# kianoosh-j/CL_MultiView_Stereo

Hardware: AMD Instinct MI355X
Metric: Mpix/s depth (1080p, 128 depth hyp, 5 views) + depth L1 vs ref (higher is better)
Workload: dtype i8 (NCC: 8-bit intensities as int8 v_dot4 operands, i32 window sums, f32 costs; SLIC / superpixel SAD / refinement in f32 with the reference's f64 promotions)

## Files before the change

### cl_multiview_stereo_amd/csrc/launch_plan.cpp

```cpp
#include "launch_plan.h"

#include <algorithm>
#include <climits>
#include <cmath>
#include <cstdlib>
#include <cstring>

extern char** environ;

namespace mvs {
namespace plan {

Tuning plan_tuning() {
  Tuning t;
  bool any = false;
  for (char** e = environ; e && *e && !any; e++) {
    const char* s = *e;
    any = s[0] == 'M' && s[1] == 'V' && s[2] == 'S' && s[3] == '_' && (s[4] == 'S' || s[4] == 'F');
  }
  if (!any) return t;
  const auto num = [](const char* name, int dflt) {
    const char* e = getenv(name);
    return e ? atoi(e) : dflt;
  };
  const auto is = [](const char* name, const char* value) {
    const char* e = getenv(name);
    return e && !strcmp(e, value);
  };
  const int wps = num("MVS_SWEEP_WPS", 0);
  t.sweep_wps = (wps == 1 || wps == 2 || wps == 4) ? wps : 0;
  t.sweep_transpose = num("MVS_SWEEP_TRANSPOSE", 2);
  t.sweep_hz = num("MVS_SWEEP_HZ", 1) != 0;
  t.sweep_ring = num("MVS_SWEEP_RING", 1) != 0;
  t.sweep_ring_fast = num("MVS_SWEEP_RING_FAST", 1) != 0;
  if (const char* kv = getenv("MVS_SAD_KERNEL")) {
    t.sad_kernel = kv;
    t.sad_named = true;
  }
  t.sad_aff = getenv("MVS_SAD_AFF") == nullptr;
  t.filter_px = is("MVS_FILTER_KERNEL", "px");
  t.filter_fb_q = num("MVS_FILTER_FB", 2);
  t.filter_fb_px = num("MVS_FILTER_FB", 4);
  t.filter_ns = num("MVS_FILTER_NS", 2);
  t.filter_bound = num("MVS_FILTER_BOUND", 1) != 0;
  t.filter_ref_order = is("MVS_FILTER_ORDER", "ref");
  t.slic_tiles9 = num("MVS_SLIC_TILES9", 0) == 1;
  t.slic_update_walk = num("MVS_SLIC_UPDATE", 1) != 0;
  return t;
}

SlicPlan plan_slic(const Tuning& t, int V, int W, int H, int S, int no_iter, int edge_enable, int search,
                   int enforce_connectivity) {
  SlicPlan p;
  p.V = V, p.W = W, p.H = H, p.S = S;
  const int mw = p.mw = map_dim(W, S), mh = p.mh = map_dim(H, S);
  float xy = 1.0f / (1.4242f * (float)S);
  float col = 15.0f / (1.7321f * 128.0f);
  p.xy = xy * xy;
  p.col = col * col;
  const bool tiles = S % kLocal == 0;
  const int cpl = p.cpl = S * 3 / kLocal;
  const int G = p.G = tiles ? cpl * cpl : (int)__builtin_ceilf((float)(S * S * 9) / (float)(kLocal * kLocal));
  const int ntx = p.ntx = (W + 15) / 16, nty = p.nty = (H + 15) / 16;
  const size_t P = (size_t)V * W * H;
  const bool l16 = !tiles && no_iter > 0 && (long)mw * mh <= 65536;
  size_t sb = tiles ? sizeof(float) * 6 * (size_t)G * mw * mh * V : 0;
  if (enforce_connectivity || edge_enable) sb = std::max(sb, sizeof(uint32_t) * P);
  if (l16) sb = std::max(sb, sizeof(uint16_t) * P);
  p.scratch_bytes = sb;

  p.steps.reserve(6 + 2 * (size_t)no_iter);
  const auto step = [&p](SlicKernel k, unsigned gx, unsigned gy, unsigned gz, unsigned block) -> SlicStep& {
    p.steps.push_back(SlicStep{k, 0, 0, 0, 0, 0, {gx, gy, gz}, block, false, false, false, false});
    return p.steps.back();
  };
  const unsigned cx = (mw + 63) / 64, px = (W + 255) / 256;
  step(kSlicInitCenters, cx, mh, V, 64);
  if (edge_enable == 1 || edge_enable == 2) {
    step(kSlicEdge, px, H, V, 256);
    if (edge_enable == 1)
      step(kSlicEdgeStore, (unsigned)std::min<long>(((long)P + 255) / 256, 8192), 1, 1, 256);
    else
      step(kSlicApplyEdge, cx, mh, V, 64);
  }
  const bool tiles4 = !search && (S == 32 || S == 64) && (long)W * H * 16 < (1L << 31) &&
                      (long)mw * mh * G * 24 < (1L << 31) && !t.slic_tiles9;
  const auto assign = [&](bool more) {
    if (tiles) {
      SlicStep& s = tiles4 ? step(kSlicAssignTiles4, (ntx + 3) / 4, nty, V, 256)
                           : step(kSlicAssignTiles9, (ntx * nty + 3) / 4, V, 1, 256);
      if (tiles4)
        s.S16 = S / 16;
      else
        s.S3 = search;
      s.labels = !more, s.part = more;
    } else {
      SlicStep& s = step(kSlicAssign, (W + kAssignTW - 1) / kAssignTW, (H + kAssignTH - 1) / kAssignTH, V, 256);
      s.S3 = search;
      s.labels = !(more && l16), s.lb16 = more && l16;
    }
  };
  const bool walk = (long)W * H * 16 < (1L << 31) && t.slic_update_walk;
  assign(no_iter > 0);
  for (int i = 0; i < no_iter; i++) {
    if (tiles) {
      step(kSlicUpdateFinalize, (mw * mh + 31) / 32, V, 1, 256).CPL = cpl == 6 ? 6 : 0;
    } else {
      SlicStep& s = step(walk ? kSlicUpdateWalk : kSlicUpdate, (mw * mh + 3) / 4, V, 1, 256);
      s.UT = G > 4 ? 4 : 1;
      s.LT = l16 ? 16 : 32;
    }
    assign(i + 1 < no_iter);
  }
  if (enforce_connectivity) {
    step(kSlicSuppress, px, H, V, 256).to_scratch = true;
    step(kSlicSuppress, px, H, V, 256);
  }
  return p;
}

SpixlSweepPlan plan_sweep_spixl(const Tuning& t, int V, int W, int H, int S, int D, const float* levels,
                                const int* vs, const int* sn, int aw, int z0, int z1, bool allow_relayout) {
  SpixlSweepPlan p;
  if (z1 <= z0) return p;
  if ((long)(W + H) * H * 16 >= (1L << 31)) {
    p.err = "superpixel sweep: image too large for 32-bit offsets";
    return p;
  }
  p.launch = true;
  p.mw = map_dim(W, S);
  p.mh = map_dim(H, S);
  const long M = (long)p.mw * p.mh;
  const bool half = D <= 32;
  int wps = (D + 63) / 64;
  wps = wps >= 3 ? 4 : wps;
  const int wps_env = half ? 0 : t.sweep_wps;
  if (wps_env) wps = wps_env;
  const int tmode = t.sweep_transpose;
  p.tstride = H;
  if (tmode > 0 && allow_relayout) {
    std::vector<int32_t> slot(4 * (size_t)V, -1);
    long units = 0;
    for (int z = z0; z < z1; z++)
      for (int k = 0; k < sn[z]; k++) {
        const int v = vs[(size_t)V * z + k];
        if (v < 0 || v >= V) continue;
        const int dx = v % aw - z % aw, dy = v / aw - z / aw;
        const int kind = dx == 0 ? 1 : tmode < 2 ? 0 : dx == dy ? 2 : dx == -dy ? 3 : 0;
        if (kind && slot[4 * v + kind] < 0 && units + W + H <= INT32_MAX) {
          slot[4 * v + kind] = (int32_t)units;
          units += kind == 1 ? W : W + H - 1;
        }
      }
    if (units > 0) {
      for (int v = 0; v < V; v++)
        for (int kind = 1; kind < 4; kind++)
          if (slot[4 * v + kind] >= 0) p.relayouts.push_back({v, kind, slot[4 * v + kind]});
      p.slot = std::move(slot);
      p.units = units;
    }
  }
  const bool relaid = p.units > 0;
  bool hz = !relaid && t.sweep_hz;
  for (int z = z0; z < z1 && hz; z++)
    for (int k = 0; k < sn[z] && hz; k++) {
      const int v = vs[(size_t)V * z + k];
      if (v / aw != z / aw) hz = false;
      const float fdxv = (float)(v % aw - z % aw);
      for (int l = 0; l < D && hz; l++) {
        const float f = levels[l] * fdxv;
        if (!(fabsf(f) < 16777216.0f) || f != truncf(f)) hz = false;
      }
    }
  bool ring = hz && !half && t.sweep_ring;
  if (ring) {
    float rng = 0.0f;
    for (int c0 = 0; c0 < D; c0 += 64) {
      float lo = levels[c0], hi = lo;
      for (int l = c0; l < std::min(D, c0 + 64); l++) {
        lo = std::min(lo, levels[l]);
        hi = std::max(hi, levels[l]);
      }
      rng = std::max(rng, hi - lo);
    }
    int mdx = 0;
    for (int z = z0; z < z1; z++)
      for (int k = 0; k < sn[z]; k++) mdx = std::max(mdx, std::abs(vs[(size_t)V * z + k] % aw - z % aw));
    if (2.0 * (S - 1) + 2.0 + (double)rng * mdx + 1.0 > (double)kSwU) ring = false;
  }
  p.form = ring ? kSweepHzRing : relaid ? kSweepRelaid : hz ? kSweepHzGather : kSweepGeneral;
  p.lps = half ? 32 : 64;
  p.wps = ring ? (wps_env ? wps_env : 1) : wps;
  const int spb = half ? 8 : 4 / p.wps;
  const long nb = (M + spb - 1) / spb;
  p.grid_x = (unsigned)(8 * ((nb + 7) / 8));
  p.grid_y = (unsigned)(z1 - z0);
  const int last[5] = {p.form, p.lps, p.wps, tmode, (int)p.relayouts.size()};
  std::copy(last, last + 5, p.last);
  return p;
}

bool sad_band_geometry(int DC, int RR, bool aff, int V, int W, int H, int D, const float* levels, const int* vs,
                       const int* sn, int aw, float bl, int z, SadPlan& p) {
  const int TH = RR - 4, PPW = DC / 8;
  const int nn = sn[z];
  const int nch = (D + DC - 1) / DC;
  const int rx = z % aw, ry = z / aw;
  constexpr int RW = sizeof(SadRec) / 4;
  std::vector<int32_t> table((size_t)std::max(1, nch * nn) * RW, 0);
  int span_x = 0;
  float span_y = 0.0f;
  for (int c = 0; c < nch; c++)
    for (int n = 0; n < nn; n++) {
      SadRec e{};
      const int view = vs[V * z + n];
      const int dx = view % aw - rx, dy = view / aw - ry;
      e.view = view;
      e.sxmin = 1 << 30;
      e.sxmax = -(1 << 30);
      e.fdymin = INFINITY;
      e.fdymax = -INFINITY;
      for (int j = 0; j < DC; j++) {
        const int dl = std::min(c * DC + j, D - 1);
        const float d = levels[dl];
        const float fdx = d * (float)dx;
        const float fdy = (bl * d) * (float)dy;
        if (fdx != std::trunc(fdx) || std::fabs(fdx) > 1e6f) return false;
        e.sx[j] = (int)fdx;
        e.fdy[j] = fdy;
        if (fdy != std::trunc(fdy) || std::fabs(fdy) > 1e6f) aff = false;
        if (c * DC + j < D) {
          e.sxmin = std::min(e.sxmin, e.sx[j]);
          e.sxmax = std::max(e.sxmax, e.sx[j]);
          e.fdymin = std::min(e.fdymin, fdy);
          e.fdymax = std::max(e.fdymax, fdy);
        }
      }
      span_x = std::max(span_x, e.sxmax - e.sxmin);
      span_y = std::max(span_y, e.fdymax - e.fdymin);
      std::memcpy(table.data() + ((size_t)c * nn + n) * RW, &e, sizeof(SadRec));
    }
  SadArgs a{};
  a.W = W; a.H = H; a.D = D; a.nn = nn; a.z = z; a.nch = nch;
  a.bw = (64 + span_x + 63) & ~63;
  a.brows = RR + (int)std::ceil(span_y) + (aff ? 0 : 1);
  const size_t lds = 16 * 2 * (size_t)a.brows * a.bw + (aff ? 0 : 4 * 2 * (size_t)DC * RR);
  if (a.bw > 64 * SB_NBLK) return false;
  if (lds > 160 * 1024 || (size_t)4 * TH * 64 * 8 > 16 * 2 * (size_t)a.brows * a.bw) return false;
  a.tiles_x = (W + SB_TW - 1) / SB_TW;
  a.ntiles = a.tiles_x * ((H + TH - 1) / TH);
  a.tiles_per_xcd = (a.ntiles + 7) / 8;
  p.band = true;
  p.TH = TH;
  p.PPW = PPW;
  p.AFF = aff;
  p.BWT = aff ? (a.bw == 64 ? 64 : 128) : 0;
  p.table = std::move(table);
  p.args = a;
  p.lds = lds;
  p.grid_x = 8 * a.tiles_per_xcd;
  p.grid_y = 1;
  return true;
}

SadPlan plan_sad(const Tuning& t, int V, int W, int H, int D, const float* levels, const int* vs, const int* sn,
                 int aw, float bl, int z) {
  SadPlan p;
  const std::string& kind = t.sad_kernel;
  const bool try2 = kind == "auto" || kind == "sys8x2", try1 = kind == "auto" || kind == "sys8";
  if (try2 && sad_band_geometry(16, 12, t.sad_aff, V, W, H, D, levels, vs, sn, aw, bl, z, p)) return p;
  if (try1 && sad_band_geometry(8, 12, t.sad_aff, V, W, H, D, levels, vs, sn, aw, bl, z, p)) return p;
  if (t.sad_named && kind != "gather") {
    p.err = "k_sad_band variant " + kind + " cannot stage this geometry (MVS_SAD_KERNEL set explicitly)";
    return p;
  }
  p.grid_x = (W + PT - 1) / PT;
  p.grid_y = (H + PT - 1) / PT;
  return p;
}

FilterPlan plan_remove_incons(const Tuning& t, int V, int W, int H, int aw, int z0, int z1, int ya, int yb,
                              bool band) {
  FilterPlan p;
  const int NR = yb - ya;
  p.PP = band ? (long)NR * W : (long)W * H;
  p.proj_off = band ? -(long)ya * W : 0;
  if (z1 <= z0 || NR <= 0) return p;
  const unsigned gx = (W + 255) / 256;
  const auto grid = [&p](unsigned x, unsigned y, unsigned z) { p.grid[0] = x, p.grid[1] = y, p.grid[2] = z; };
  const bool off32 = (long)V * W * H * 4 < (1L << 31);
  if (V <= 8 && off32) {
    p.kernel = kFilterSel8;
    grid(gx, NR, z1 - z0);
  } else if (V <= 16) {
    p.kernel = kFilterPx16_8;
    grid(gx, NR, 1);
  } else if (V <= 32 && off32 && !t.filter_px) {
    p.kernel = kFilterQ;
    p.FB = t.filter_fb_q == 4 ? 4 : 2;
    p.NS = t.filter_ns == 1 ? 1 : 2;
    p.ROWB = aw % p.FB == 0;
    p.RM = !t.filter_ref_order;
    p.inb = (V % aw == 0 && t.filter_bound) ? 1 : 0;
    const unsigned tx = (W + 63) / 64, groups = (z1 - z0 + kFilterRG - 1) / kFilterRG;
    if (p.RM)
      grid(tx * groups, NR, 1);
    else
      grid(tx, NR, groups);
    p.block = 64 * kFilterRG;
  } else if (V <= 32) {
    p.kernel = kFilterPx32;
    p.FB = t.filter_fb_px == 4 ? 4 : t.filter_fb_px == 2 ? 2 : 8;
    grid(gx, NR, 1);
  } else if (V <= 64 && off32) {
    p.kernel = kFilterSel64;
    grid(gx, NR, z1 - z0);
  } else {
    p.kernel = kFilterPlain;
    grid(gx, NR, z1 - z0);
  }
  return p;
}

SgmPlan plan_sgm(int W, int H, int D, int path) {
  SgmPlan p;
  if (W < 1 || H < 1 || D < 1 || path < 0 || path > 3) {
    p.err = "sgm: bad dimensions or path";
    return p;
  }
  if (D > kSgmMaxD) {
    p.err = "sgm: more than 16384 levels";
    return p;
  }
  const bool vertical = path >= 2;
  p.rev = path & 1;
  p.n = vertical ? H : W;
  p.lines = vertical ? W : H;
// ... 106 lines not shown
```

### cl_multiview_stereo_amd/csrc/launch_plan.h

```cpp
#pragma once
#include <cstddef>
#include <cstdint>
#include <string>
#include <vector>

namespace mvs {

inline int map_dim(int n, int S) {
  return (int)__builtin_ceilf((float)n / (float)S);
}

constexpr int kLocal = 16;
constexpr int kAssignTW = 64, kAssignTH = 16;

constexpr int kSwU = 336;

struct SweepArgs {
  int V, W, H, mw, mh, D, aw, z;
  float bl;
};
constexpr float SB_INIT = 1000000.0f;

constexpr int SB_TW = 60;
constexpr int SB_NBLK = 2;
struct SadArgs {
  int W, H, D, nn, z;
  int tiles_x, ntiles, tiles_per_xcd, nch;
  int bw, brows;
};
struct alignas(16) SadRec {
  int view, sxmin, sxmax, pad0;
  float fdymin, fdymax;
  int pad1[2];
  int sx[16];
  float fdy[16];
};
static_assert(sizeof(SadRec) == 160, "SadRec is uploaded as 40 int32 words");
constexpr int PT = 32;

constexpr int kFilterRG = 4;

namespace plan {

struct Tuning {
  bool slic_tiles9 = false;
  bool slic_update_walk = true;
  int sweep_wps = 0;
  int sweep_transpose = 2;
  bool sweep_hz = true;
  bool sweep_ring = true;
  bool sweep_ring_fast = true;
  std::string sad_kernel = "auto";
  bool sad_named = false;
  bool sad_aff = true;
  bool filter_px = false;
  int filter_fb_q = 2;
  int filter_fb_px = 4;
  int filter_ns = 2;
  bool filter_bound = true;
  bool filter_ref_order = false;
};
Tuning plan_tuning();

enum SlicKernel {
  kSlicInitCenters, kSlicEdge, kSlicEdgeStore, kSlicApplyEdge,
  kSlicAssign,
  kSlicAssignTiles9,
  kSlicAssignTiles4,
  kSlicUpdateFinalize,
  kSlicUpdateWalk,
  kSlicUpdate,
  kSlicSuppress
};
struct SlicStep {
  SlicKernel kernel;
  int S3, S16, CPL, UT, LT;
  unsigned grid[3], block;
  bool labels;
  bool lb16;
  bool part;
  bool to_scratch;
};
struct SlicPlan {
  int V = 0, W = 0, H = 0, S = 0;
  int mw = 0, mh = 0;
  float xy = 0, col = 0;
  int G = 0, cpl = 0, ntx = 0, nty = 0;
  size_t scratch_bytes = 0;
  std::vector<SlicStep> steps;
};
SlicPlan plan_slic(const Tuning& t, int V, int W, int H, int S, int no_iter, int edge_enable, int search,
                   int enforce_connectivity);

constexpr int kSweepGeneral = 0, kSweepHzGather = 1, kSweepHzRing = 2, kSweepRelaid = 3;
struct SpixlRelayout {
  int view, kind, slot;
};
struct SpixlSweepPlan {
  const char* err = nullptr;
  bool launch = false;
  int form = 0, lps = 64, wps = 1;
  int mw = 0, mh = 0;
  unsigned grid_x = 0, grid_y = 0;
  std::vector<int32_t> slot;
  std::vector<SpixlRelayout> relayouts;
  long units = 0, tstride = 0;
  int last[5] = {0, 0, 0, 0, 0};
};
SpixlSweepPlan plan_sweep_spixl(const Tuning& t, int V, int W, int H, int S, int D, const float* levels,
                                const int* vs, const int* sn, int aw, int z0, int z1, bool allow_relayout);

struct SadPlan {
  bool band = false;
  int TH = 0, PPW = 0, AFF = 0, BWT = 0;
  std::vector<int32_t> table;
  SadArgs args{};
  size_t lds = 0;
  unsigned grid_x = 0, grid_y = 1;
  std::string err;
};
bool sad_band_geometry(int DC, int RR, bool aff, int V, int W, int H, int D, const float* levels, const int* vs,
                       const int* sn, int aw, float bl, int z, SadPlan& p);
SadPlan plan_sad(const Tuning& t, int V, int W, int H, int D, const float* levels, const int* vs, const int* sn,
                 int aw, float bl, int z);

enum FilterKernel { kFilterNone, kFilterSel8, kFilterPx16_8, kFilterQ, kFilterPx32, kFilterSel64, kFilterPlain };
struct FilterPlan {
  FilterKernel kernel = kFilterNone;
  int FB = 0, NS = 0, ROWB = 0, RM = 0;
  int inb = 0;
  unsigned grid[3] = {0, 1, 1}, block = 256;
  long PP = 0;
  long proj_off = 0;
};
FilterPlan plan_remove_incons(const Tuning& t, int V, int W, int H, int aw, int z0, int z1, int ya, int yb,
                              bool band);

constexpr int kSgmLanes = 0, kSgmColumns = 1;
constexpr int kSgmMaxLpl = 16;
constexpr int kSgmLanesOneWave = 64 * kSgmMaxLpl;
constexpr int kSgmColumnsLpw = 16;
constexpr int kSgmColumnsMaxD = 16 * kSgmColumnsLpw;
constexpr int kSgmMaxD = 16 * kSgmLanesOneWave;
struct SgmPlan {
  const char* err = nullptr;
  int form = kSgmLanes;
  int lpl = 1;
  int waves = 1;
  bool vec = false;
  int n = 0, lines = 0;
  int sstride = 0, lstride = 0;
  int sx = 0;
  bool rev = false;
  unsigned grid = 0, block = 0;
  size_t lds = 0;
};
SgmPlan plan_sgm(int W, int H, int D, int path);

constexpr int kSgmSheared = 2;
constexpr int sgm_diag_x0(int g, int lane, int H, int sx) { return sx > 0 ? 64 * g - (H - 1) + lane : 64 * g + lane; }
constexpr int sgm_diag_ylo(int g, int W, int H, int sx) {
  const int y = sx > 0 ? H - 1 - 64 * g - 63 : 64 * g - (W - 1);
  return y > 0 ? y : 0;
}
constexpr int sgm_diag_yhi(int g, int W, int H, int sx) {
  const int y = sx > 0 ? W + H - 2 - 64 * g : 64 * g + 63;
  return y < H - 1 ? y : H - 1;
}
struct SgmDiagLine {
  int first, n;
};
constexpr SgmDiagLine sgm_diag_line(int W, int H, int sx, int l) {
  const int c = l - (H - 1);
  const int xt = sx > 0 ? (c > 0 ? c : 0) : (l < W ? l : W - 1);
  const int yt = sx > 0 ? (c < 0 ? -c : 0) : (l < W ? 0 : l - (W - 1));
  const int nx = sx > 0 ? W - xt : xt + 1, ny = H - yt;
  return {yt * W + xt, nx < ny ? nx : ny};
}
SgmPlan plan_sgm_diag(int W, int H, int D, int path);

constexpr int kSgmMaxBatch = 65535;
constexpr int kSgm16MaxD = kSgmColumnsMaxD;
constexpr int kSgm16MaxCost = 4094, kSgm16MaxP = 4095;
constexpr int kSgmPiece = 4, kSgm16Piece = 8;
struct SgmCost {
  int piece;
  int max_d;
  bool unsupported;
};
constexpr SgmCost kSgmF32 = {kSgmPiece, kSgmMaxD, false}, kSgmU16 = {kSgm16Piece, kSgm16MaxD, true};
struct SgmBatchPlan {
  const char* err = nullptr;
  bool unsupported = false;
  unsigned grid_y = 0;
  bool vec_ok = false;
};
SgmBatchPlan plan_sgm_batch(SgmCost cost, int W, int H, int D, int N, uintptr_t vol_addr, size_t vol_stride,
                            uintptr_t agg_addr, size_t agg_stride);
constexpr bool sgm_piece_vec_ok(int piece, int N, uintptr_t vol_addr, size_t vol_stride, uintptr_t agg_addr,
                                size_t agg_stride) {
  return ((vol_addr ^ agg_addr) & 15) == 0 && (N == 1 || ((vol_stride - agg_stride) & (size_t)(piece - 1)) == 0);
}
constexpr int sgm_piece_phase(int piece, uintptr_t line_addr) {
  return (int)((line_addr / (uintptr_t)(16 / piece)) & (uintptr_t)(piece - 1));
}
constexpr int sgm_piece_elem(int piece, int ph, int x) { return (x + ph) & (piece - 1); }
constexpr bool sgm_piece_inside(int piece, int ph, int x, int n) {
  return x - sgm_piece_elem(piece, ph, x) >= 0 && x - sgm_piece_elem(piece, ph, x) + piece - 1 < n;
}

}
}
```

### cl_multiview_stereo_amd/csrc/sweep.hip

```cpp
#include <algorithm>
#include <type_traits>

#include "mvs_internal.h"
#include "wave.h"

namespace mvs {
namespace {

__global__ __launch_bounds__(256) void k_boundary(const float* __restrict__ spixl,
                                                  const uint32_t* __restrict__ labels, int W, int H, int S, int mw,
                                                  int mh, uint8_t* __restrict__ rep) {
  const int lane = threadIdx.x & 63;
  const long s = (long)blockIdx.x * 4 + (threadIdx.x >> 6);
  const int z = blockIdx.y;
  const long M = (long)mw * mh, P = (long)W * H;
  if (s >= M) return;
  const float* sp = spixl + 8 * (z * M + s);
  int cx = (int)sp[1], cy = (int)sp[2];
  if (cx < S) cx += (S - cx);
  if (cx + S > W) cx -= S;
  if (cy < S) cy += (S - cy);
  if (cy + S > H) cy -= S;
  const uint32_t id = (uint32_t)s;
  const uint32_t* L = labels + z * P;
  const int k = lane >> 3, j = lane & 7;
  const int dx = k < 3 ? -1 : (k < 5 ? 0 : 1);
  const int dy = (k == 0 || k == 3 || k == 5) ? -1 : ((k == 1 || k == 6) ? 0 : 1);
  int d = 0;
  for (int i0 = 1; i0 < S; i0 += 32) {
    uint32_t v[4];
    bool in[4];
#pragma unroll
    for (int m = 0; m < 4; m++) {
      const int i = i0 + j + 8 * m, xx = cx + dx * i, yy = cy + dy * i;
      in[m] = i < S && xx >= 0 && xx < W && yy >= 0 && yy < H;
      v[m] = L[in[m] ? (long)yy * W + xx : 0];
    }
#pragma unroll
    for (int m = 0; m < 4; m++)
      if (in[m] && v[m] == id) d = i0 + j + 8 * m - 1;
  }
  d = max(d, __shfl_xor(d, 1));
  d = max(d, __shfl_xor(d, 2));
  d = max(d, __shfl_xor(d, 4));
  uint32_t w = (uint32_t)(d & 0xff) << (8 * (k & 3));
  w |= __shfl_xor(w, 8);
  w |= __shfl_xor(w, 16);
  const uint32_t hi = __shfl(w, 32);
  if (lane == 0) *(uint2*)(rep + 8 * (z * M + s)) = make_uint2(w, hi);
}

__device__ __forceinline__ float tap_ad(const float4& A, const u32x3& bv) {
  float t0, t1, t2, r;
  asm("v_sub_f32 %0, %1, %2" : "=v"(t0) : "v"(A.x), "v"(__uint_as_float(bv.x)));
  asm("v_sub_f32 %0, %1, %2" : "=v"(t1) : "v"(A.y), "v"(__uint_as_float(bv.y)));
  asm("v_add_f32 %0, |%1|, |%2|" : "=v"(r) : "v"(t0), "v"(t1));
  asm("v_sub_f32 %0, %1, %2" : "=v"(t2) : "v"(A.z), "v"(__uint_as_float(bv.z)));
  asm("v_add_f32 %0, %1, |%2|" : "=v"(r) : "v"(r), "v"(t2));
  return r;
}
__device__ __forceinline__ float tap_acc(float val, float ad, bool in) {
  float v30, t;
  asm("v_add_f32 %0, 0x41f00000, %1" : "=v"(v30) : "v"(val));
  asm("v_add_f32 %0, 0xc1f00000, %1" : "=v"(t) : "v"(v30));
  asm("v_add_f32 %0, %1, %2" : "=v"(t) : "v"(t), "v"(ad));
  return in ? t : v30;
}
template <int LPS, bool TL, bool HZ = false>
__global__ __launch_bounds__(256) void k_sweep_spixl(const float4* __restrict__ lab, float* __restrict__ spixl,
                                                     const uint8_t* __restrict__ rep,
                                                     const float* __restrict__ levels, const int* __restrict__ vs,
                                                     const int* __restrict__ sn, SweepArgs a, int wps,
                                                     const float4* __restrict__ labT,
                                                     const int* __restrict__ tslot, long tstride) {
  __shared__ float4 refc[8][25];
  __shared__ float2 refxy[8][25];
  __shared__ float wbest[4];
  __shared__ int wbi[4];
  const int lane = threadIdx.x & 63, w = threadIdx.x >> 6;
  const int ll = lane & (LPS - 1);
  const int spb = LPS == 64 ? 4 / wps : 8, h = LPS == 64 ? w % wps : 0;
  const int slot = LPS == 64 ? w / wps : 2 * w + (lane >> 5);
  const int z = a.z + blockIdx.y;
  const long M = (long)a.mw * a.mh, P = (long)a.W * a.H;
  const long nb = (M + spb - 1) / spb, per = (nb + 7) / 8;
  const long blk = (long)(blockIdx.x & 7) * per + (blockIdx.x >> 3);
  const long s = blk * spb + slot;
  const bool active = blk < nb && s < M && slot < spb;
  const long idx = z * M + (active ? s : 0);
  const uint8_t* dr = rep + 8 * idx;
  int bl_ = max((int)dr[0], max((int)dr[1], (int)dr[2]));
  int br_ = max((int)dr[5], max((int)dr[6], (int)dr[7]));
  int bt_ = max((int)dr[0], max((int)dr[3], (int)dr[5]));
  int bb_ = max((int)dr[2], max((int)dr[4], (int)dr[7]));
  float stx = (float)fmax(1.0, 0.25 * (double)(float)(bl_ + br_));
  float sty = (float)fmax(1.0, 0.25 * (double)(float)(bt_ + bb_));
  float cx = spixl[8 * idx + 1], cy = spixl[8 * idx + 2];
  const float4* labz = lab + (long)z * P;
  if (ll < 25 && (LPS == 32 || h == 0)) {
    int i = ll / 5 - 2, j = ll % 5 - 2;
    int xr = (int)(cx + (float)i * stx);
    int yr = (int)(cy + (float)j * sty);
    bool in = xr >= 0 && yr >= 0 && xr < a.W && yr < a.H;
    if (HZ)
      refxy[slot][ll] = make_float2(__int_as_float(in ? xr : -(1 << 30)), __int_as_float(in ? yr * a.W : 0));
    else
      refxy[slot][ll] = make_float2(in ? (float)xr : -1.0e9f, (float)yr);
    refc[slot][ll] = in ? labz[(long)yr * a.W + xr] : make_float4(0.f, 0.f, 0.f, 0.f);
  }
  __syncthreads();
  int rx = z % a.aw, ry = z / a.aw;
  int nn = sn[z];
  float best = SB_INIT;
  int bi = 0x7fffffff;
  for (int dl = ll + LPS * h; dl < a.D; dl += LPS * wps) {
    float d = levels[dl];
    float mn = SB_INIT;
    for (int n = 0; n < nn; n++) {
      int view = vs[a.V * z + n];
      int vx = view % a.aw, vy = view / a.aw;
      float fdx = d * (float)(vx - rx);
      float fdy = (a.bl * d) * (float)(vy - ry);
      const int ddx = vx - rx, ddy = vy - ry;
      if (HZ) {
        const int sh = (int)fdx;
        const __amdgpu_buffer_rsrc_t rs = buf_rsrc(lab + (long)view * P, (int)(P * 16));
        float val = 0.0f;
#pragma unroll 5
        for (int t = 0; t < 25; t++) {
          const float2 rf = refxy[slot][t];
          const int xp = __float_as_int(rf.x) - sh;
          const bool in = (unsigned)xp < (unsigned)a.W;
          const unsigned bo = (unsigned)(__float_as_int(rf.y) + xp) << 4;
          const u32x3 bv = __builtin_amdgcn_raw_buffer_load_b96(rs, (int)bo, 0, 0);
          val = tap_acc(val, tap_ad(refc[slot][t], bv), in);
        }
        if (val < mn) mn = val;
        continue;
      }
      const int kind = !TL ? 0 : ddx == 0 ? 1 : ddx == ddy ? 2 : ddx == -ddy ? 3 : 0;
      const int ts = TL && kind ? tslot[4 * view + kind] : -1;
      const float4* labv = TL && ts >= 0 ? labT + (long)ts * tstride : lab + (long)view * P;
      const __amdgpu_buffer_rsrc_t rs = buf_rsrc(labv, 0x7fffffff);
      const int sxs = !TL || ts < 0 ? 1 : a.H;
      const int sys = !TL || ts < 0 ? a.W : kind == 1 ? 1 : kind == 2 ? 1 - a.H : a.H + 1;
      const int off = TL && ts >= 0 && kind == 2 ? (a.H - 1) * a.H : 0;
      float val = 0.0f;
#pragma unroll 5
      for (int t = 0; t < 25; t++) {
        const float2 r = refxy[slot][t];
        const int xp = (int)(r.x - fdx);
        const int yp = (int)(r.y - fdy);
        const bool in = (unsigned)xp < (unsigned)a.W && (unsigned)yp < (unsigned)a.H;
        const int bo = in ? (off + yp * sys + xp * sxs) * 16 : 0;
        const u32x3 bv = __builtin_amdgcn_raw_buffer_load_b96(rs, bo, 0, 0);
        const float3 B = make_float3(__uint_as_float(bv.x), __uint_as_float(bv.y), __uint_as_float(bv.z));
        const float4 A = refc[slot][t];
        float ad = fabsf(A.x - B.x) + fabsf(A.y - B.y);
        ad = ad + fabsf(A.z - B.z);
        const float v30 = val + 30.0f;
        val = in ? (v30 - 30.0f) + ad : v30;
      }
      if (val < mn) mn = val;
    }
    if (mn < best) {
      best = mn;
      bi = dl;
    }
  }
#pragma unroll
  for (int o = LPS / 2; o >= 1; o >>= 1) {
    float ob = __shfl_xor(best, o, 64);
    int oi = __shfl_xor(bi, o, 64);
    if (ob < best || (ob == best && oi < bi)) {
      best = ob;
      bi = oi;
    }
  }
  if (LPS == 32) {
    if (active && ll == 0) spixl[8 * idx + 7] = (bi != 0x7fffffff && best < SB_INIT) ? levels[bi] : 0.0f;
    return;
  }
  if (lane == 0) {
    wbest[w] = best;
    wbi[w] = bi;
  }
  __syncthreads();
  if (active && h == 0 && lane == 0) {
    for (int k = 1; k < wps; k++) {
      const float ob = wbest[w + k];
      const int oi = wbi[w + k];
      if (ob < best || (ob == best && oi < bi)) {
        best = ob;
        bi = oi;
      }
    }
    spixl[8 * idx + 7] = (bi != 0x7fffffff && best < SB_INIT) ? levels[bi] : 0.0f;
  }
}

__device__ __forceinline__ float wave_min_f(float v) {
  v = fminf(v, __shfl_xor(v, 32));
  v = fminf(v, __shfl_xor(v, 16));
  v = fminf(v, __shfl_xor(v, 8));
  v = fminf(v, __shfl_xor(v, 4));
  v = fminf(v, __shfl_xor(v, 2));
  v = fminf(v, __shfl_xor(v, 1));
  return __int_as_float(__builtin_amdgcn_readfirstlane(__float_as_int(v)));
}
__device__ __forceinline__ float tap_acc_in(float val, float ad) {
  float t;
  asm("v_add_f32 %0, 0x41f00000, %1" : "=v"(t) : "v"(val));
  asm("v_add_f32 %0, 0xc1f00000, %1" : "=v"(t) : "v"(t));
  asm("v_add_f32 %0, %1, %2" : "=v"(t) : "v"(t), "v"(ad));
  return t;
}
template <int OFF>
__device__ __forceinline__ void ring_taps5(const unsigned (&ra)[5], unsigned rb, u32x3 (&Bv)[5], f32x4 (&Av)[5]) {
  asm volatile(
      "ds_read_b96 %0, %10 offset:%16\n\t"
      "ds_read_b96 %1, %11 offset:%16\n\t"
      "ds_read_b96 %2, %12 offset:%16\n\t"
      "ds_read_b96 %3, %13 offset:%16\n\t"
      "ds_read_b96 %4, %14 offset:%16\n\t"
      "ds_read_b128 %5, %15\n\t"
      "ds_read_b128 %6, %15 offset:80\n\t"
      "ds_read_b128 %7, %15 offset:160\n\t"
      "ds_read_b128 %8, %15 offset:240\n\t"
      "ds_read_b128 %9, %15 offset:320\n\t"
      "s_waitcnt lgkmcnt(0)"
      : "=&v"(Bv[0]), "=&v"(Bv[1]), "=&v"(Bv[2]), "=&v"(Bv[3]), "=&v"(Bv[4]), "=&v"(Av[0]), "=&v"(Av[1]),
        "=&v"(Av[2]), "=&v"(Av[3]), "=&v"(Av[4])
      : "v"(ra[0]), "v"(ra[1]), "v"(ra[2]), "v"(ra[3]), "v"(ra[4]), "v"(rb), "i"(OFF)
      : "memory");
}
template <int WPS>
__global__ __launch_bounds__(256) void k_sweep_spixl_ring(const float4* __restrict__ lab, float* __restrict__ spixl,
                                                          const uint8_t* __restrict__ rep,
                                                          const float* __restrict__ levels, const int* __restrict__ vs,
                                                          const int* __restrict__ sn, SweepArgs a, int fast) {
  constexpr int SPB = 4 / WPS;
  constexpr unsigned kSlotB = kSwU * 16u;
  __shared__ __align__(16) float4 ring[4][2][kSwU];
  __shared__ float4 refc[SPB][25];
  __shared__ int rxr[SPB][5], ryr[SPB][5];
  __shared__ unsigned rvm[SPB];
  __shared__ float wbest[4];
  __shared__ int wbi[4];
  const int lane = threadIdx.x & 63, w = __builtin_amdgcn_readfirstlane(threadIdx.x >> 6);
  const int h = w % WPS, slot = w / WPS;
  const int z = a.z + blockIdx.y;
  const long M = (long)a.mw * a.mh, P = (long)a.W * a.H;
  const long nbk = (M + SPB - 1) / SPB, per = (nbk + 7) / 8;
  const long blk = (long)(blockIdx.x & 7) * per + (blockIdx.x >> 3);
  const long s = blk * SPB + slot;
  const bool active = blk < nbk && s < M;
  const long idx = z * M + (active ? s : 0);
  if (h == 0) {
    const uint8_t* dr = rep + 8 * idx;
    const int bl_ = max((int)dr[0], max((int)dr[1], (int)dr[2]));
    const int br_ = max((int)dr[5], max((int)dr[6], (int)dr[7]));
    const int bt_ = max((int)dr[0], max((int)dr[3], (int)dr[5]));
    const int bb_ = max((int)dr[2], max((int)dr[4], (int)dr[7]));
    const float stx = (float)fmax(1.0, 0.25 * (double)(float)(bl_ + br_));
    const float sty = (float)fmax(1.0, 0.25 * (double)(float)(bt_ + bb_));
    const float cx = spixl[8 * idx + 1], cy = spixl[8 * idx + 2];
    const int i = lane / 5 - 2, j = lane % 5 - 2;
    const int xr = (int)(cx + (float)i * stx);
    const int yr = (int)(cy + (float)j * sty);
    const bool in = lane < 25 && xr >= 0 && yr >= 0 && xr < a.W && yr < a.H;
    if (lane < 25) {
      float4 rc = in ? lab[(long)z * P + (long)yr * a.W + xr] : make_float4(0.f, 0.f, 0.f, 0.f);
      rc.w = __int_as_float(in ? xr : -(1 << 30));
      refc[slot][lane] = rc;
      if (j == -2) rxr[slot][i + 2] = xr;
      if (i == -2) ryr[slot][j + 2] = yr;
    }
    const unsigned long long bal = __ballot(in);
    if (lane == 0) rvm[slot] = (unsigned)bal;
  }
  __syncthreads();
  const unsigned vm = __builtin_amdgcn_readfirstlane(rvm[slot]);
  int xr[5], yr[5];
#pragma unroll
  for (int q = 0; q < 5; q++) {
    xr[q] = __builtin_amdgcn_readfirstlane(rxr[slot][q]);
    yr[q] = __builtin_amdgcn_readfirstlane(ryr[slot][q]);
  }
  int xlo = 1 << 30, xhi = -(1 << 30);
#pragma unroll
  for (int q = 0; q < 5; q++)
    if ((vm >> (5 * q)) & 0x1fu) {
      xlo = min(xlo, xr[q]);
      xhi = max(xhi, xr[q]);
    }
  const int rx = z % a.aw;
  const unsigned ring_base = (unsigned)(uintptr_t)(lds_ptr_t)&ring[w][0][0];
  const unsigned refc_base = (unsigned)(uintptr_t)(lds_ptr_t)&refc[slot][0];
  const int nn = sn[z];
  float best = SB_INIT;
  int bi = 0x7fffffff;
  for (int p0 = 64 * h; p0 < a.D; p0 += 64 * WPS) {
    const int dl = p0 + lane;
    const bool act = dl < a.D;
    const float d = levels[act ? dl : a.D - 1];
    const float dlo = wave_min_f(d), dhi = -wave_min_f(-d);
    const float4* pl_s = lab;
    int ulo_s = 0, U_s = 0, sh_s = 0, vo_s = 0;
    bool whole_s = false;
    auto open_nb = [&](int n) {
      const int view = vs[a.V * z + n];
      const float fdx = (float)(view % a.aw - rx);
      sh_s = (int)(d * fdx);
      const int s0 = (int)(dlo * fdx), s1 = (int)(dhi * fdx);
      const int shmin = min(s0, s1), shmax = max(s0, s1);
      const int lo = xlo - shmax, hi = xhi - shmin;
      ulo_s = max(lo, 0);
      const int U = min(hi, a.W - 1) - ulo_s + 1;
      whole_s = lo >= 0 && hi < a.W && U <= kSwU;
      U_s = min(U, kSwU);
      vo_s = 16 * min(lane, max(U_s, 1) - 1);
      pl_s = lab + (long)view * P;
    };
    auto stage = [&](int j, int sl) -> int {
      if (U_s <= 0 || !((vm >> j) & 0x108421u)) return 0;
      const __amdgpu_buffer_rsrc_t rs = buf_rsrc(pl_s, (int)(P * 16));
      const int ro = (yr[j] * a.W + ulo_s) * 16;
      const int np = (U_s + 63) >> 6;
      for (int q = 0; q < np; q++) {
        const int c0 = U_s >= 64 ? min(q * 64, U_s - 64) : 0;
        __builtin_amdgcn_raw_ptr_buffer_load_lds(rs, (lds_ptr_t)&ring[w][sl][c0], 16, vo_s, ro + 16 * c0, 0, 0);
      }
      return np;
    };
    float mn = SB_INIT;
    if (nn > 0) {
      open_nb(0);
      int pcn = stage(0, 0);
      pcn = stage(1, 1);
      int ulo_c = ulo_s, sh_c = sh_s;
      bool whole_c = whole_s;
      for (int n = 0; n < nn; n++) {
        const int par = n & 1;
        auto stage_ahead = [&](int j) {
          int pc2 = 0;
          if (j < 3 || n + 1 < nn) {
            if (j == 3) open_nb(n + 1);
            pc2 = stage(j < 3 ? j + 2 : j - 3, (par + j) & 1);
          }
          pcn = pc2;
        };
        auto whole_rows = [&](auto PAR) -> float {
          unsigned ra[5];
#pragma unroll
          for (int i = 0; i < 5; i++) ra[i] = ring_base + (unsigned)(xr[i] - sh_c - ulo_c) * 16u;
          float ad[25];
#pragma unroll
          for (int j = 0; j < 5; j++) {
            wait_vm(5 * n + j + 1 < 5 * nn ? pcn : 0);
            u32x3 Bv[5];
            f32x4 Av[5];
            const unsigned rb = refc_base + (unsigned)j * 16u;
            if ((decltype(PAR)::value + j) & 1)
              ring_taps5<(int)kSlotB>(ra, rb, Bv, Av);
            else
              ring_taps5<0>(ra, rb, Bv, Av);
            stage_ahead(j);
#pragma unroll
            for (int i = 0; i < 5; i++) {
              const int t = 5 * i + j;
              ad[t] = tap_ad(make_float4(Av[i].x, Av[i].y, Av[i].z, 0.f), Bv[i]);
            }
          }
          float val = 0.0f;
#pragma unroll
          for (int t = 0; t < 25; t++) val = tap_acc_in(val, ad[t]);
          return val;
        };
        if (fast && vm == 0x1ffffffu && whole_c) {
          const float val = par ? whole_rows(std::integral_constant<int, 1>()) : whole_rows(std::integral_constant<int, 0>());
          mn = val < mn ? val : mn;
          if (n + 1 < nn) ulo_c = ulo_s, sh_c = sh_s, whole_c = whole_s;
          continue;
        }
        float ad[25];
#pragma unroll
        for (int j = 0; j < 5; j++) {
          const int k = 5 * n + j;
          wait_vm(k + 1 < 5 * nn ? pcn : 0);
          int xp[5];
          unsigned ra[5];
#pragma unroll
          for (int i = 0; i < 5; i++) {
            xp[i] = ((vm >> (5 * i + j)) & 1u ? xr[i] : -(1 << 30)) - sh_c;
            const bool in = (unsigned)xp[i] < (unsigned)a.W;
            ra[i] = ring_base + (unsigned)(k & 1) * kSlotB + (in ? (unsigned)(xp[i] - ulo_c) * 16u : 0u);
          }
          const unsigned rb = refc_base + (unsigned)j * 16u;
          u32x3 Bv[5];
          f32x4 Av[5];
          asm volatile(
              "ds_read_b96 %0, %10\n\t"
              "ds_read_b96 %1, %11\n\t"
              "ds_read_b96 %2, %12\n\t"
              "ds_read_b96 %3, %13\n\t"
              "ds_read_b96 %4, %14\n\t"
              "ds_read_b128 %5, %15\n\t"
              "ds_read_b128 %6, %15 offset:80\n\t"
              "ds_read_b128 %7, %15 offset:160\n\t"
              "ds_read_b128 %8, %15 offset:240\n\t"
              "ds_read_b128 %9, %15 offset:320\n\t"
              "s_waitcnt lgkmcnt(0)"
              : "=&v"(Bv[0]), "=&v"(Bv[1]), "=&v"(Bv[2]), "=&v"(Bv[3]), "=&v"(Bv[4]), "=&v"(Av[0]), "=&v"(Av[1]),
                "=&v"(Av[2]), "=&v"(Av[3]), "=&v"(Av[4])
              : "v"(ra[0]), "v"(ra[1]), "v"(ra[2]), "v"(ra[3]), "v"(ra[4]), "v"(rb)
              : "memory");
#pragma unroll
          for (int i = 0; i < 5; i++) {
            const bool in = (unsigned)xp[i] < (unsigned)a.W;
            const float v = tap_ad(make_float4(Av[i].x, Av[i].y, Av[i].z, 0.f), Bv[i]);
            ad[5 * i + j] = in ? v : -1.0f;
          }
          stage_ahead(j);
        }
        float val = 0.0f;
#pragma unroll
        for (int t = 0; t < 25; t++) val = tap_acc(val, ad[t], ad[t] >= 0.0f);
        mn = val < mn ? val : mn;
        if (n + 1 < nn) ulo_c = ulo_s, sh_c = sh_s, whole_c = whole_s;
      }
    }
    if (act && mn < best) {
      best = mn;
      bi = dl;
    }
  }
#pragma unroll
  for (int o = 32; o >= 1; o >>= 1) {
    const float ob = __shfl_xor(best, o, 64);
    const int oi = __shfl_xor(bi, o, 64);
    if (ob < best || (ob == best && oi < bi)) {
      best = ob;
      bi = oi;
    }
  }
  if (lane == 0) {
    wbest[w] = best;
    wbi[w] = bi;
  }
  __syncthreads();
  if (active && h == 0 && lane == 0) {
    for (int k = 1; k < WPS; k++) {
      const float ob = wbest[w + k];
      const int oi = wbi[w + k];
      if (ob < best || (ob == best && oi < bi)) {
        best = ob;
        bi = oi;
      }
    }
    spixl[8 * idx + 7] = (bi != 0x7fffffff && best < SB_INIT) ? levels[bi] : 0.0f;
  }
}

template <int KIND>
__global__ __launch_bounds__(256) void k_relayout_lab(const float4* __restrict__ lab, int W, int H, int view,
                                                      float4* __restrict__ out) {
  __shared__ float4 t[32][33];
  const int x0 = blockIdx.x * 32, y0 = blockIdx.y * 32, tx = threadIdx.x & 31, ty = threadIdx.x >> 5;
  const float4* src = lab + (long)view * W * H;
#pragma unroll
  for (int k = 0; k < 4; k++) {
    const int y = y0 + ty + 8 * k, x = x0 + tx;
    if (x < W && y < H) t[ty + 8 * k][tx] = src[(long)y * W + x];
  }
  __syncthreads();
  if (KIND == 1) {
#pragma unroll
    for (int k = 0; k < 4; k++) {
      const int x = x0 + ty + 8 * k, y = y0 + tx;
      if (x < W && y < H) out[(long)x * H + y] = t[tx][ty + 8 * k];
    }
    return;
  }
  for (int d0 = 0; d0 < 63; d0 += 8) {
    const int dd = d0 + ty, yl = tx;
    const int xl = KIND == 2 ? yl + dd - 31 : dd - yl;
    const int x = x0 + xl, y = y0 + yl;
    if (dd < 63 && xl >= 0 && xl < 32 && x < W && y < H)
      out[KIND == 2 ? (long)(x - y + H - 1) * H + y : (long)(x + y) * H + y] = t[yl][xl];
  }
}

}

int launch_boundary(hipStream_t s, int V, int W, int H, int S, const float* spixl, const uint32_t* labels,
                    uint8_t* rep) {
  int mw = map_dim(W, S), mh = map_dim(H, S);
  hipLaunchKernelGGL(k_boundary, dim3((mw * mh + 3) / 4, V), dim3(256), 0, s, spixl, labels, W, H, S, mw, mh, rep);
  MVS_LAUNCH_CHECK("k_boundary");
  return 0;
}

int launch_sweep_spixl(mvs_ctx* ctx, int V, int W, int H, int S, const float* lab, float* spixl,
                       const uint8_t* rep, const float* levels, int D, const int* vs, const int* sn, int aw,
                       float bl, int z0, int z1) {
  const plan::Tuning t = plan::plan_tuning();
  const auto planned = [&](bool relayout) {
    return plan::plan_sweep_spixl(t, V, W, H, S, D, ctx->h_levels.data(), ctx->h_vs.data(), ctx->h_sn.data(), aw, z0,
                                  z1, relayout);
  };
  plan::SpixlSweepPlan p = planned(true);
  if (p.err) return arg_fail(p.err);
  if (!p.launch) return 0;
  hipStream_t s = ctx->stream;
  const float4* labT = nullptr;
  const int* tslot = nullptr;
  if (p.units > 0) {
    int rc = 0;
    float4* buf = (float4*)scratch(ctx, (size_t)p.units * p.tstride * sizeof(float4), &rc);
    if (rc == MVS_E_NOMEM) {
      (void)hipGetLastError();
      p = planned(false);
    } else if (rc) {
      return rc;
    } else {
      tslot = plan_upload(ctx, p.slot, &rc);
      if (rc) return rc;
      labT = buf;
      const dim3 tg((W + 31) / 32, (H + 31) / 32);
      static constexpr void (*relayout[3])(const float4*, int, int, int, float4*) = {k_relayout_lab<1>, k_relayout_lab<2>,
                                                                                     k_relayout_lab<3>};
      for (const plan::SpixlRelayout& r : p.relayouts)
        hipLaunchKernelGGL(relayout[r.kind - 1], tg, dim3(256), 0, s, (const float4*)lab, W, H, r.view,
                           buf + (long)r.slot * p.tstride);
      MVS_LAUNCH_CHECK("k_relayout_lab");
    }
  }
  SweepArgs a{V, W, H, p.mw, p.mh, D, aw, z0, bl};
  const dim3 g(p.grid_x, p.grid_y);
  if (p.form == plan::kSweepHzRing) {
    static constexpr void (*ring[3])(const float4*, float*, const uint8_t*, const float*, const int*, const int*,
                                     SweepArgs, int) = {k_sweep_spixl_ring<1>, k_sweep_spixl_ring<2>, k_sweep_spixl_ring<4>};
    hipLaunchKernelGGL(ring[p.wps == 1 ? 0 : p.wps == 2 ? 1 : 2], g, dim3(256), 0, s, (const float4*)lab, spixl, rep,
                       levels, vs, sn, a, (int)t.sweep_ring_fast);
    MVS_LAUNCH_CHECK("k_sweep_spixl_ring");
  } else {
    const bool half = p.lps == 32;
    const auto kern = p.form == plan::kSweepRelaid     ? (half ? k_sweep_spixl<32, true> : k_sweep_spixl<64, true>)
                      : p.form == plan::kSweepHzGather ? (half ? k_sweep_spixl<32, false, true> : k_sweep_spixl<64, false, true>)
                                                       : (half ? k_sweep_spixl<32, false> : k_sweep_spixl<64, false>);
    hipLaunchKernelGGL(kern, g, dim3(256), 0, s, (const float4*)lab, spixl, rep, levels, vs, sn, a, p.wps, labT, tslot,
                       p.tstride);
    MVS_LAUNCH_CHECK("k_sweep_spixl");
  }
  std::copy(p.last, p.last + 5, ctx->sweep_last);
  return 0;
}

}
```

Measured before the change: 6133.

## Pair two depth passes per staged neighbor window in ring superpixel sweep

The ring sweep kernel now processes two depth-hypothesis passes together when their combined shift window fits the staged LDS ring. Each staged neighbor row is reused for both depth sets, with one shared read of the reference taps. This halves the global-to-LDS staging per pair and amortizes the loop overhead. The cost is doubled register arrays (bd, Cv), which may lower occupancy, and more complex control flow with a fallback mode that restages when the union window is too wide.

```diff
diff --git a/cl_multiview_stereo_amd/csrc/launch_plan.cpp b/cl_multiview_stereo_amd/csrc/launch_plan.cpp
--- a/cl_multiview_stereo_amd/csrc/launch_plan.cpp
+++ b/cl_multiview_stereo_amd/csrc/launch_plan.cpp
@@ -33,6 +33,7 @@
   t.sweep_hz = num("MVS_SWEEP_HZ", 1) != 0;
   t.sweep_ring = num("MVS_SWEEP_RING", 1) != 0;
   t.sweep_ring_fast = num("MVS_SWEEP_RING_FAST", 1) != 0;
+  t.sweep_ring_pair = num("MVS_SWEEP_RING_PAIR", 1) != 0;
   if (const char* kv = getenv("MVS_SAD_KERNEL")) {
     t.sad_kernel = kv;
     t.sad_named = true;
diff --git a/cl_multiview_stereo_amd/csrc/launch_plan.h b/cl_multiview_stereo_amd/csrc/launch_plan.h
--- a/cl_multiview_stereo_amd/csrc/launch_plan.h
+++ b/cl_multiview_stereo_amd/csrc/launch_plan.h
@@ -50,6 +50,7 @@
   bool sweep_hz = true;
   bool sweep_ring = true;
   bool sweep_ring_fast = true;
+  bool sweep_ring_pair = true;
   std::string sad_kernel = "auto";
   bool sad_named = false;
   bool sad_aff = true;
diff --git a/cl_multiview_stereo_amd/csrc/sweep.hip b/cl_multiview_stereo_amd/csrc/sweep.hip
--- a/cl_multiview_stereo_amd/csrc/sweep.hip
+++ b/cl_multiview_stereo_amd/csrc/sweep.hip
@@ -234,6 +234,32 @@
       : "v"(ra[0]), "v"(ra[1]), "v"(ra[2]), "v"(ra[3]), "v"(ra[4]), "v"(rb), "i"(OFF)
       : "memory");
 }
+template <int OFF>
+__device__ __forceinline__ void ring_taps5x2(const unsigned (&ra)[5], const unsigned (&rc)[5], unsigned rb,
+                                             u32x3 (&Bv)[5], u32x3 (&Cv)[5], f32x4 (&Av)[5]) {
+  asm volatile(
+      "ds_read_b96 %0, %15 offset:%26\n\t"
+      "ds_read_b96 %1, %16 offset:%26\n\t"
+      "ds_read_b96 %2, %17 offset:%26\n\t"
+      "ds_read_b96 %3, %18 offset:%26\n\t"
+      "ds_read_b96 %4, %19 offset:%26\n\t"
+      "ds_read_b96 %5, %20 offset:%26\n\t"
+      "ds_read_b96 %6, %21 offset:%26\n\t"
+      "ds_read_b96 %7, %22 offset:%26\n\t"
+      "ds_read_b96 %8, %23 offset:%26\n\t"
+      "ds_read_b96 %9, %24 offset:%26\n\t"
+      "ds_read_b128 %10, %25\n\t"
+      "ds_read_b128 %11, %25 offset:80\n\t"
+      "ds_read_b128 %12, %25 offset:160\n\t"
+      "ds_read_b128 %13, %25 offset:240\n\t"
+      "ds_read_b128 %14, %25 offset:320\n\t"
+      "s_waitcnt lgkmcnt(0)"
+      : "=&v"(Bv[0]), "=&v"(Bv[1]), "=&v"(Bv[2]), "=&v"(Bv[3]), "=&v"(Bv[4]), "=&v"(Cv[0]), "=&v"(Cv[1]),
+        "=&v"(Cv[2]), "=&v"(Cv[3]), "=&v"(Cv[4]), "=&v"(Av[0]), "=&v"(Av[1]), "=&v"(Av[2]), "=&v"(Av[3]), "=&v"(Av[4])
+      : "v"(ra[0]), "v"(ra[1]), "v"(ra[2]), "v"(ra[3]), "v"(ra[4]), "v"(rc[0]), "v"(rc[1]), "v"(rc[2]), "v"(rc[3]),
+        "v"(rc[4]), "v"(rb), "i"(OFF)
+      : "memory");
+}
 template <int WPS>
 __global__ __launch_bounds__(256) void k_sweep_spixl_ring(const float4* __restrict__ lab, float* __restrict__ spixl,
                                                           const uint8_t* __restrict__ rep,
@@ -300,27 +326,49 @@
   const int nn = sn[z];
   float best = SB_INIT;
   int bi = 0x7fffffff;
-  for (int p0 = 64 * h; p0 < a.D; p0 += 64 * WPS) {
-    const int dl = p0 + lane;
-    const bool act = dl < a.D;
-    const float d = levels[act ? dl : a.D - 1];
-    const float dlo = wave_min_f(d), dhi = -wave_min_f(-d);
+  const bool pair = (fast & 2) != 0;
+  fast &= 1;
+  constexpr int kPass = 64 * WPS;
+  for (int p0 = 64 * h; p0 < a.D;) {
+    const bool two = pair && p0 + kPass < a.D;
+    const int dl0 = p0 + lane, dl1 = dl0 + kPass;
+    const bool act0 = dl0 < a.D, act1 = two && dl1 < a.D;
+    const float d0 = levels[act0 ? dl0 : a.D - 1], d1 = levels[act1 ? dl1 : a.D - 1];
+    const float dlo0 = wave_min_f(d0), dhi0 = -wave_min_f(-d0);
+    float dlo1 = dlo0, dhi1 = dhi0;
+    if (two) dlo1 = wave_min_f(d1), dhi1 = -wave_min_f(-d1);
     const float4* pl_s = lab;
-    int ulo_s = 0, U_s = 0, sh_s = 0, vo_s = 0;
+    int ulo_s = 0, U_s = 0, shA_s = 0, shB_s = 0, vo_s = 0, md_s = 0, n_s = 0;
     bool whole_s = false;
-    auto open_nb = [&](int n) {
+    auto open_unit = [&](int n, bool second) {
       const int view = vs[a.V * z + n];
       const float fdx = (float)(view % a.aw - rx);
-      sh_s = (int)(d * fdx);
-      const int s0 = (int)(dlo * fdx), s1 = (int)(dhi * fdx);
-      const int shmin = min(s0, s1), shmax = max(s0, s1);
-      const int lo = xlo - shmax, hi = xhi - shmin;
-      ulo_s = max(lo, 0);
-      const int U = min(hi, a.W - 1) - ulo_s + 1;
-      whole_s = lo >= 0 && hi < a.W && U <= kSwU;
+      const int sh0 = (int)(d0 * fdx), sh1 = (int)(d1 * fdx);
+      auto window = [&](float lo_d, float hi_d) -> int {
+        const int s0 = (int)(lo_d * fdx), s1 = (int)(hi_d * fdx);
+        const int shmin = min(s0, s1), shmax = max(s0, s1);
+        const int lo = xlo - shmax, hi = xhi - shmin;
+        ulo_s = max(lo, 0);
+        const int U = min(hi, a.W - 1) - ulo_s + 1;
+        whole_s = lo >= 0 && hi < a.W && U <= kSwU;
+        return U;
+      };
+      int U = 0;
+      if (second) {
+        md_s = 1, shA_s = sh1;
+        U = window(dlo1, dhi1);
+      } else {
+        md_s = 0, shA_s = sh0, shB_s = sh1;
+        if (two) {
+          U = window(fminf(dlo0, dlo1), fmaxf(dhi0, dhi1));
+          md_s = U <= kSwU ? 2 : 3;
+        }
+        if (md_s != 2) U = window(dlo0, dhi0);
+      }
       U_s = min(U, kSwU);
       vo_s = 16 * min(lane, max(U_s, 1) - 1);
       pl_s = lab + (long)view * P;
+      n_s = n;
     };
     auto stage = [&](int j, int sl) -> int {
       if (U_s <= 0 || !((vm >> j) & 0x108421u)) return 0;
@@ -333,107 +381,152 @@
       }
       return np;
     };
-    float mn = SB_INIT;
+    float mn0 = SB_INIT, mn1 = SB_INIT;
     if (nn > 0) {
-      open_nb(0);
+      open_unit(0, false);
       int pcn = stage(0, 0);
       pcn = stage(1, 1);
-      int ulo_c = ulo_s, sh_c = sh_s;
+      int ulo_c = ulo_s, shA_c = shA_s, shB_c = shB_s, md_c = md_s, n_c = n_s;
       bool whole_c = whole_s;
-      for (int n = 0; n < nn; n++) {
-        const int par = n & 1;
+      for (int par = 0;; par ^= 1) {
+        const bool more = md_c == 3 || n_c + 1 < nn;
         auto stage_ahead = [&](int j) {
           int pc2 = 0;
-          if (j < 3 || n + 1 < nn) {
-            if (j == 3) open_nb(n + 1);
+          if (j < 3 || more) {
+            if (j == 3) {
+              if (md_s == 3)
+                open_unit(n_s, true);
+              else
+                open_unit(n_s + 1, false);
+            }
             pc2 = stage(j < 3 ? j + 2 : j - 3, (par + j) & 1);
           }
           pcn = pc2;
         };
-        auto whole_rows = [&](auto PAR) -> float {
-          unsigned ra[5];
-#pragma unroll
-          for (int i = 0; i < 5; i++) ra[i] = ring_base + (unsigned)(xr[i] - sh_c - ulo_c) * 16u;
-          float ad[25];
+        float valA = 0.0f, valB = 0.0f;
+        auto whole_rows = [&](auto PAR, auto BOTH) {
+          constexpr bool kBoth = decltype(BOTH)::value;
+          unsigned ra[5], rc[5];
+#pragma unroll
+          for (int i = 0; i < 5; i++) {
+            ra[i] = ring_base + (unsigned)(xr[i] - shA_c - ulo_c) * 16u;
+            rc[i] = ring_base + (unsigned)(xr[i] - shB_c - ulo_c) * 16u;
+          }
+          float ad[25], bd[25];
 #pragma unroll
           for (int j = 0; j < 5; j++) {
-            wait_vm(5 * n + j + 1 < 5 * nn ? pcn : 0);
-            u32x3 Bv[5];
+            wait_vm(j < 4 || more ? pcn : 0);
+            u32x3 Bv[5], Cv[5];
             f32x4 Av[5];
             const unsigned rb = refc_base + (unsigned)j * 16u;
-            if ((decltype(PAR)::value + j) & 1)
-              ring_taps5<(int)kSlotB>(ra, rb, Bv, Av);
+            if constexpr (kBoth) {
+              if ((decltype(PAR)::value + j) & 1)
+                ring_taps5x2<(int)kSlotB>(ra, rc, rb, Bv, Cv, Av);
+              else
+                ring_taps5x2<0>(ra, rc, rb, Bv, Cv, Av);
+            } else {
+              if ((decltype(PAR)::value + j) & 1)
+                ring_taps5<(int)kSlotB>(ra, rb, Bv, Av);
+              else
+                ring_taps5<0>(ra, rb, Bv, Av);
+            }
+            stage_ahead(j);
+#pragma unroll
+            for (int i = 0; i < 5; i++) {
+              const int t = 5 * i + j;
+              const float4 A = make_float4(Av[i].x, Av[i].y, Av[i].z, 0.f);
+              ad[t] = tap_ad(A, Bv[i]);
+              if constexpr (kBoth) bd[t] = tap_ad(A, Cv[i]);
+            }
+          }
+#pragma unroll
+          for (int t = 0; t < 25; t++) valA = tap_acc_in(valA, ad[t]);
+          if constexpr (kBoth) {
+#pragma unroll
+            for (int t = 0; t < 25; t++) valB = tap_acc_in(valB, bd[t]);
+          }
+        };
+        auto general_rows = [&](auto BOTH) {
+          constexpr bool kBoth = decltype(BOTH)::value;
+          float ad[25], bd[25];
+#pragma unroll
+          for (int j = 0; j < 5; j++) {
+            wait_vm(j < 4 || more ? pcn : 0);
+            const unsigned sb = ring_base + (unsigned)((par + j) & 1) * kSlotB;
+            int xp[5], xq[5];
+            unsigned ra[5], rc[5];
+#pragma unroll
+            for (int i = 0; i < 5; i++) {
+              const int x0 = (vm >> (5 * i + j)) & 1u ? xr[i] : -(1 << 30);
+              xp[i] = x0 - shA_c;
+              xq[i] = x0 - shB_c;
+              ra[i] = sb + ((unsigned)xp[i] < (unsigned)a.W ? (unsigned)(xp[i] - ulo_c) * 16u : 0u);
+              rc[i] = sb + ((unsigned)xq[i] < (unsigned)a.W ? (unsigned)(xq[i] - ulo_c) * 16u : 0u);
+            }
+            const unsigned rb = refc_base + (unsigned)j * 16u;
+            u32x3 Bv[5], Cv[5];
+            f32x4 Av[5];
+            if constexpr (kBoth)
+              ring_taps5x2<0>(ra, rc, rb, Bv, Cv, Av);
             else
               ring_taps5<0>(ra, rb, Bv, Av);
+#pragma unroll
+            for (int i = 0; i < 5; i++) {
+              const float4 A = make_float4(Av[i].x, Av[i].y, Av[i].z, 0.f);
+              const float v = tap_ad(A, Bv[i]);
+              ad[5 * i + j] = (unsigned)xp[i] < (unsigned)a.W ? v : -1.0f;
+              if constexpr (kBoth) {
+                const float u = tap_ad(A, Cv[i]);
+                bd[5 * i + j] = (unsigned)xq[i] < (unsigned)a.W ? u : -1.0f;
+              }
+            }
             stage_ahead(j);
-#pragma unroll
-            for (int i = 0; i < 5; i++) {
-              const int t = 5 * i + j;
-              ad[t] = tap_ad(make_float4(Av[i].x, Av[i].y, Av[i].z, 0.f), Bv[i]);
-            }
           }
-          float val = 0.0f;
-#pragma unroll
-          for (int t = 0; t < 25; t++) val = tap_acc_in(val, ad[t]);
-          return val;
+#pragma unroll
+          for (int t = 0; t < 25; t++) valA = tap_acc(valA, ad[t], ad[t] >= 0.0f);
+          if constexpr (kBoth) {
+#pragma unroll
+            for (int t = 0; t < 25; t++) valB = tap_acc(valB, bd[t], bd[t] >= 0.0f);
+          }
         };
+        using std::false_type;
+        using std::true_type;
         if (fast && vm == 0x1ffffffu && whole_c) {
-          const float val = par ? whole_rows(std::integral_constant<int, 1>()) : whole_rows(std::integral_constant<int, 0>());
-          mn = val < mn ? val : mn;
-          if (n + 1 < nn) ulo_c = ulo_s, sh_c = sh_s, whole_c = whole_s;
-          continue;
+          if (md_c == 2) {
+            if (par)
+              whole_rows(std::integral_constant<int, 1>(), true_type());
+            else
+              whole_rows(std::integral_constant<int, 0>(), true_type());
+          } else {
+            if (par)
+              whole_rows(std::integral_constant<int, 1>(), false_type());
+            else
+              whole_rows(std::integral_constant<int, 0>(), false_type());
+          }
+        } else {
+          if (md_c == 2)
+            general_rows(true_type());
+          else
+            general_rows(false_type());
         }
-        float ad[25];
-#pragma unroll
-        for (int j = 0; j < 5; j++) {
-          const int k = 5 * n + j;
-          wait_vm(k + 1 < 5 * nn ? pcn : 0);
-          int xp[5];
-          unsigned ra[5];
-#pragma unroll
-          for (int i = 0; i < 5; i++) {
-            xp[i] = ((vm >> (5 * i + j)) & 1u ? xr[i] : -(1 << 30)) - sh_c;
-            const bool in = (unsigned)xp[i] < (unsigned)a.W;
-            ra[i] = ring_base + (unsigned)(k & 1) * kSlotB + (in ? (unsigned)(xp[i] - ulo_c) * 16u : 0u);
-          }
-          const unsigned rb = refc_base + (unsigned)j * 16u;
-          u32x3 Bv[5];
-          f32x4 Av[5];
-          asm volatile(
-              "ds_read_b96 %0, %10\n\t"
-              "ds_read_b96 %1, %11\n\t"
-              "ds_read_b96 %2, %12\n\t"
-              "ds_read_b96 %3, %13\n\t"
-              "ds_read_b96 %4, %14\n\t"
-              "ds_read_b128 %5, %15\n\t"
-              "ds_read_b128 %6, %15 offset:80\n\t"
-              "ds_read_b128 %7, %15 offset:160\n\t"
-              "ds_read_b128 %8, %15 offset:240\n\t"
-              "ds_read_b128 %9, %15 offset:320\n\t"
-              "s_waitcnt lgkmcnt(0)"
-              : "=&v"(Bv[0]), "=&v"(Bv[1]), "=&v"(Bv[2]), "=&v"(Bv[3]), "=&v"(Bv[4]), "=&v"(Av[0]), "=&v"(Av[1]),
-                "=&v"(Av[2]), "=&v"(Av[3]), "=&v"(Av[4])
-              : "v"(ra[0]), "v"(ra[1]), "v"(ra[2]), "v"(ra[3]), "v"(ra[4]), "v"(rb)
-              : "memory");
-#pragma unroll
-          for (int i = 0; i < 5; i++) {
-            const bool in = (unsigned)xp[i] < (unsigned)a.W;
-            const float v = tap_ad(make_float4(Av[i].x, Av[i].y, Av[i].z, 0.f), Bv[i]);
-            ad[5 * i + j] = in ? v : -1.0f;
-          }
-          stage_ahead(j);
-        }
-        float val = 0.0f;
-#pragma unroll
-        for (int t = 0; t < 25; t++) val = tap_acc(val, ad[t], ad[t] >= 0.0f);
-        mn = val < mn ? val : mn;
-        if (n + 1 < nn) ulo_c = ulo_s, sh_c = sh_s, whole_c = whole_s;
+        if (md_c == 1)
+          mn1 = valA < mn1 ? valA : mn1;
+        else
+          mn0 = valA < mn0 ? valA : mn0;
+        if (md_c == 2) mn1 = valB < mn1 ? valB : mn1;
+        if (!more) break;
+        ulo_c = ulo_s, shA_c = shA_s, shB_c = shB_s, md_c = md_s, n_c = n_s, whole_c = whole_s;
       }
     }
-    if (act && mn < best) {
-      best = mn;
-      bi = dl;
-    }
+    if (act0 && mn0 < best) {
+      best = mn0;
+      bi = dl0;
+    }
+    if (act1 && mn1 < best) {
+      best = mn1;
+      bi = dl1;
+    }
+    p0 += two ? 2 * kPass : kPass;
   }
 #pragma unroll
   for (int o = 32; o >= 1; o >>= 1) {
@@ -542,7 +635,7 @@
     static constexpr void (*ring[3])(const float4*, float*, const uint8_t*, const float*, const int*, const int*,
                                      SweepArgs, int) = {k_sweep_spixl_ring<1>, k_sweep_spixl_ring<2>, k_sweep_spixl_ring<4>};
     hipLaunchKernelGGL(ring[p.wps == 1 ? 0 : p.wps == 2 ? 1 : 2], g, dim3(256), 0, s, (const float4*)lab, spixl, rep,
-                       levels, vs, sn, a, (int)t.sweep_ring_fast);
+                       levels, vs, sn, a, (int)t.sweep_ring_fast | (t.sweep_ring_pair ? 2 : 0));
     MVS_LAUNCH_CHECK("k_sweep_spixl_ring");
   } else {
     const bool half = p.lps == 32;
```

New measurement: 6171, median of 6. No clear change (+0.6%).
